# Dao-AILab/flash-attention

Hardware: AMD Instinct MI355X
Metric: attention_fwd_tflops (higher is better)
Workload: dtype bf16; 1 GPU; BASELINE config 3: B=4 H=32 S=4096 D=128 bf16 causal, forward (flash_attn_func path, fa_fwd via C ABI); batch=4, heads=32, seqlen=4096, head_dim=128, causal=True, parallelism=replicas x1

## Files before the change

flash-attention_amd/csrc/fa_fwd_w64.hip:

```cpp
#include <cstddef>
#include <cstdio>
#include <cstdlib>
#include <type_traits>

#include "fa_device.h"
#include "fa_kernel_params.h"
#include "fa_launch.h"
#include "fa_fwd_w64_regs.h"
#define FA_W64_CLOB FA_W64_ACC_CLOBBERS
#include "fa_w64_asm.h"


#define FA_W64_AH 3
#define FA_W64_KDMA_G0 0
#define FA_W64_KDMA_GS 2
#define FA_W64_VDMA_G0 1
#define FA_W64_VDMA_GS 2

namespace fa {

template <int D> FA_DEVINL constexpr int k_swz_w(int row) { return D == 128 ? (row & 15) : ((row >> 1) & 7); }
template <int D> FA_DEVINL constexpr int v_swz_w(int row) { return D == 128 ? (row & 3) : ((row >> 1) & 1); }

#define FA_W64_MFMA(E_) (std::is_same<E_, __bf16>::value ? "v_mfma_f32_32x32x16_bf16" : "v_mfma_f32_32x32x16_f16")
constexpr int W64_Q_BASE = 128;
template <typename E, int F> FA_DEVINL void mfma_s_first(f32x16& d, u32x4 a, const f32x16& c) {
  if constexpr (std::is_same<E, __bf16>::value)
    asm volatile("v_mfma_f32_32x32x16_bf16 %0, %1, a[%c3:%c4], %2" : "=&v"(d) : "v"(a), "v"(c), "i"(W64_Q_BASE + 4 * F), "i"(W64_Q_BASE + 4 * F + 3) : FA_W64_ACC_CLOBBERS);
  else
    asm volatile("v_mfma_f32_32x32x16_f16 %0, %1, a[%c3:%c4], %2" : "=&v"(d) : "v"(a), "v"(c), "i"(W64_Q_BASE + 4 * F), "i"(W64_Q_BASE + 4 * F + 3) : FA_W64_ACC_CLOBBERS);
}
template <typename E, int F> FA_DEVINL void mfma_s_acc(f32x16& d, u32x4 a) {
  if constexpr (std::is_same<E, __bf16>::value)
    asm volatile("v_mfma_f32_32x32x16_bf16 %0, %1, a[%c2:%c3], %0" : "+v"(d) : "v"(a), "i"(W64_Q_BASE + 4 * F), "i"(W64_Q_BASE + 4 * F + 3) : FA_W64_ACC_CLOBBERS);
  else
    asm volatile("v_mfma_f32_32x32x16_f16 %0, %1, a[%c2:%c3], %0" : "+v"(d) : "v"(a), "i"(W64_Q_BASE + 4 * F), "i"(W64_Q_BASE + 4 * F + 3) : FA_W64_ACC_CLOBBERS);
}
template <typename E, int T> FA_DEVINL void mfma_o_acc(u32x4 a, u32x4 b) {
  if constexpr (std::is_same<E, __bf16>::value)
    asm volatile("v_mfma_f32_32x32x16_bf16 a[%c2:%c3], %0, %1, a[%c2:%c3]" : : "v"(a), "v"(b), "i"(16 * T), "i"(16 * T + 15) : FA_W64_ACC_CLOBBERS);
  else
    asm volatile("v_mfma_f32_32x32x16_f16 a[%c2:%c3], %0, %1, a[%c2:%c3]" : : "v"(a), "v"(b), "i"(16 * T), "i"(16 * T + 15) : FA_W64_ACC_CLOBBERS);
}
template <typename E, int D, int FEAT = 0, bool PAGED = false, bool DENSE = false>
__global__ void __launch_bounds__(256, 1) fa_fwd_w64_kernel(const FwdK p) {
  constexpr bool ALIBI = FEAT == FEAT_ALIBI;
  static_assert(!PAGED || FEAT == 0, "the paged variant serves plain attention");
  static_assert(!DENSE || (FEAT == 0 && !PAGED), "the dense variant serves plain attention on contiguous keys / values");
  constexpr bool SOFTCAP = FEAT == FEAT_CAP;
  constexpr bool DROP = FEAT == FEAT_DROP;
  constexpr bool DESC = ALIBI;
  static_assert(FEAT == 0 || FEAT == FEAT_ALIBI || FEAT == FEAT_CAP || FEAT == FEAT_DROP, "feature variants of this schedule: none, causal ALiBi, softcap, dropout");
  using T = ElemTraits<E>;
  using V8 = typename T::v8;
  constexpr int NW = 4, QB = 2, BM = NW * 64, BN = 64, CPR = D / 8;
  constexpr int ROW_BYTES = D * 2;
  constexpr int TILE_BYTES = BN * ROW_BYTES;
  constexpr int KS = D / 16;
  constexpr int DB = D / 32;
  static_assert(D == 64 || D == 128, "head dims built natively: 64, 128");
  constexpr float kLn2 = 0.6931471805599453f;

  extern __shared__ __attribute__((aligned(16))) char smem[];
  char FA_LDS* lds = (char FA_LDS*)smem;
  constexpr int STAGE_BYTES = BM * (ROW_BYTES + 16);
  constexpr int Q_OFF = (4 * TILE_BYTES > STAGE_BYTES ? 4 * TILE_BYTES : STAGE_BYTES + 1023) / 1024 * 1024;

  const int tid = threadIdx.x;
  const int lane = tid & 63;
  const int wave = __builtin_amdgcn_readfirstlane(tid >> 6);
  const int hi = lane >> 5, qi = lane & 31;

  const int d_row = lane / CPR, d_pc = lane % CPR;
  constexpr int RPD = 1024 / ROW_BYTES;

// ... 252 lines not shown
  {
    q_in_lds = -1;
    if (nxt_id_ok && fill_blk(nxt)) {
      asm volatile("s_waitcnt lgkmcnt(0)" ::: "memory");
      qn_srd = q_srd_of(nxt); qn_done = 0;
      qn_per_iter = n_tiles >= QDMA ? 1 : n_tiles >= QDMA / 2 ? 2 : n_tiles >= QDMA / 4 ? 4 : QDMA;
      if (n_tiles == 0) { dma_q(qn_srd); lds_dma_wait_all(); qn_done = QDMA; }
      q_in_lds = vb + (int)gridDim.x;
    }
  }
  auto q_trickle = [&]() __attribute__((always_inline)) {
    if (qn_done < QDMA) {
#pragma unroll 1
      for (int j = 0; j < qn_per_iter; ++j) dma_q_piece(qn_srd, qn_done + j);
      qn_done += qn_per_iter;
    }
  };

  const int kbase = qi * ROW_BYTES + ((hi ^ k_swz_w<D>(qi)) << 4);
  const int tr_i = lane & 15, tr_half = (lane >> 4) & 1;
  const int tr_rr = tr_i >> 2, tr_cc = tr_i & 3;
  const int vbase = (4 * hi + tr_rr) * ROW_BYTES + (v_swz_w<D>(tr_rr) << 6) + tr_half * 32 + tr_cc * 8;
  int ka[KS], va[DB];
#pragma unroll
  for (int ks = 0; ks < KS; ++ks) ka[ks] = kbase ^ (ks << 5);
#pragma unroll
  for (int db = 0; db < DB; ++db) va[db] = vbase ^ (db << 6);

  {
    u32x4 zf = {0u, 0u, 0u, 0u};
    asm volatile("" : "+v"(zf));
    acc_zero_tuples_mfma<0>(zf, std::make_integer_sequence<int, 2 * DB>{});
  }
  float m_run[QB], l_run[QB][2], o_lag[QB];
  float thr_l[QB];
  float capc = 0.f, cap_m2c = 0.f, capoff[QB] = {0.f, 0.f};
  if constexpr (SOFTCAP) {
    capc = __builtin_bit_cast(float, __builtin_amdgcn_readfirstlane(__builtin_bit_cast(int, p.softcap * 1.4426950408889634f)));
    cap_m2c = -2.f * capc;
    capoff[0] = capc; capoff[1] = capc;
  }
  unsigned drop_kr[7] = {0u, 0u, 0u, 0u, 0u, 0u, 0u}, drop_thr = 255u, drop_row[QB] = {0u, 0u};
  if constexpr (DROP) {
    const unsigned k0_ = (unsigned)__builtin_amdgcn_readfirstlane((int)drop_bh_key(p.rng, b * p.h + h));
#pragma unroll
    for (int r = 0; r < 7; ++r) drop_kr[r] = k0_ + (unsigned)r * 0x9E3779B9u;
    drop_thr = (unsigned)__builtin_amdgcn_readfirstlane((int)p.drop_thr8);
#pragma unroll
    for (int qb = 0; qb < QB; ++qb) drop_row[qb] = (unsigned)(w_row0 + 32 * qb + qi);
  }
  constexpr float kCapTiny = 7.888609052210118e-31f;
  unsigned long long lag_mask = 0ull;
  f32x16 negm[QB];
  int arel[QB] = {0, 0};
  if constexpr (ALIBI) {
#pragma unroll
    for (int qb = 0; qb < QB; ++qb) arel[qb] = 4 * hi - (w_row0 + 32 * qb + qi) - shift;
  }
  const float ainc = slope2 * 32.f;
  f32x16 sA[QB], sB[QB];
  u32x4 pfA[QB][2], pfB[QB][2];
#pragma unroll
  for (int qb = 0; qb < QB; ++qb) {
    m_run[qb] = -INFINITY; l_run[qb][0] = 0.f; l_run[qb][1] = 0.f; o_lag[qb] = 1.f; thr_l[qb] = -INFINITY;
#pragma unroll
    for (int r = 0; r < 16; ++r) { negm[qb][r] = ALIBI ? slope2 * (float)(arel[qb] + step_key(0) + acc_row(r, 0)) : 0.f; sA[qb][r] = -INFINITY; sB[qb][r] = -INFINITY; }
#pragma unroll
    for (int t = 0; t < 2; ++t) { pfA[qb][t] = u32x4{0u, 0u, 0u, 0u}; pfB[qb][t] = u32x4{0u, 0u, 0u, 0u}; }
  }

  auto rescale = [&](auto qbc, bool grow, float tmax, f32x16& s_nxt) __attribute__((always_inline)) {
    constexpr int qb = decltype(qbc)::value;
    const float m_base = (m_run[qb] == -INFINITY) ? 0.f : m_run[qb];
    const float m_upd = grow ? (tmax + m_base) : m_run[qb];
    const float m_safe = (m_upd == -INFINITY) ? 0.f : m_upd;
    const float alpha = (grow && m_run[qb] != -INFINITY) ? fast_exp2(m_run[qb] - m_safe) : 1.f;
    const float delta = m_safe - m_base;
    m_run[qb] = m_upd;
    thr_l[qb] = grow ? thr : thr_l[qb];
    l_run[qb][0] *= alpha;
    l_run[qb][1] *= alpha;
    const float neg = -m_safe;
    if constexpr (SOFTCAP) capoff[qb] = capc - m_safe;
#pragma unroll
    for (int r = 0; r < (SOFTCAP ? 0 : 16); ++r) {
      float sv = s_nxt[r], nv = negm[qb][r];
      if constexpr (ALIBI) asm volatile("v_sub_f32 %0, %0, %2\n\tv_sub_f32 %1, %1, %2" : "+v"(sv), "+v"(nv) : "v"(delta), "v"(neg));
      else asm volatile("v_sub_f32 %0, %0, %2\n\tv_mov_b32 %1, %3" : "+v"(sv), "+v"(nv) : "v"(delta), "v"(neg));
      s_nxt[r] = sv;
      negm[qb][r] = nv;
    }
    if (lag_mask != 0ull) acc_scale_range<16 * DB * qb>(o_lag[qb], std::make_integer_sequence<int, 16 * DB>{});
    o_lag[qb] = alpha;
  };
  auto decide_and_rescale = [&](const float (&tmax)[QB], f32x16 (&s_nxt)[QB]) __attribute__((always_inline)) {
    unsigned long long grow_mask;
    asm volatile("v_cmp_gt_f32 vcc, %1, %2\n\tv_cmp_gt_f32 %0, %3, %4\n\ts_or_b64 %0, %0, vcc"
                 : "=&s"(grow_mask) : "v"(tmax[0]), "v"(thr_l[0]), "v"(tmax[1]), "v"(thr_l[1]) : "vcc");
    if (__builtin_expect((grow_mask | lag_mask) != 0ull, 0)) {
      const bool g0 = tmax[0] > thr_l[0], g1 = tmax[1] > thr_l[1];
      mfma_drain_acc();
      rescale(ICw<0>{}, g0, tmax[0], s_nxt[0]);
      rescale(ICw<1>{}, g1, tmax[1], s_nxt[1]);
      lag_mask = __builtin_amdgcn_ballot_w64(o_lag[0] != 1.f || o_lag[1] != 1.f) != 0ull ? ~0ull : 0ull;
    }
  };
  auto set_mask = [&](int i_step) __attribute__((always_inline)) {
    const int k0m = step_key(i_step);
    float ninf = -INFINITY;
    asm volatile("" : "+v"(ninf));
    static_for<QB>([&](auto mqc) __attribute__((always_inline)) {
      constexpr int mq = decltype(mqc)::value;
      float nb = (SOFTCAP || m_run[mq] == -INFINITY) ? 0.f : -m_run[mq];
      const int rel_hi = min(lim_hi[mq] - k0m - 4 * hi, 31), rel_lo = max(lim_lo[mq] - k0m - 4 * hi, 0);
      const unsigned ones = (rel_hi - rel_lo >= 31) ? 0xffffffffu : ((2u << ((rel_hi - rel_lo) & 31)) - 1u);
      unsigned bits = (rel_hi >= rel_lo) ? (ones << (rel_lo & 31)) : 0u;
      if constexpr (ALIBI) nb += slope2 * (float)(arel[mq] + k0m);
      asm volatile("" : "+v"(nb), "+v"(bits));
#pragma unroll
      for (int r = 0; r < 16; r += 4) {
        float n0 = negm[mq][r], n1 = negm[mq][r + 1], n2 = negm[mq][r + 2], n3 = negm[mq][r + 3];
        unsigned t0, t1;
        if constexpr (ALIBI) {
          const float v0 = nb + slope2 * (float)acc_row(r, 0), v1 = nb + slope2 * (float)acc_row(r + 1, 0);
          const float v2 = nb + slope2 * (float)acc_row(r + 2, 0), v3 = nb + slope2 * (float)acc_row(r + 3, 0);
          asm volatile("v_bfe_i32 %4, %6, %c11, 1\n\tv_bfe_i32 %5, %6, %c12, 1\n\tv_bfi_b32 %0, %4, %7, %15\n\tv_bfi_b32 %1, %5, %8, %15\n\t"
                       "v_bfe_i32 %4, %6, %c13, 1\n\tv_bfe_i32 %5, %6, %c14, 1\n\tv_bfi_b32 %2, %4, %9, %15\n\tv_bfi_b32 %3, %5, %10, %15"
                       : "+v"(n0), "+v"(n1), "+v"(n2), "+v"(n3), "=&v"(t0), "=&v"(t1)
                       : "v"(bits), "v"(v0), "v"(v1), "v"(v2), "v"(v3), "i"(acc_row(r, 0)), "i"(acc_row(r + 1, 0)), "i"(acc_row(r + 2, 0)), "i"(acc_row(r + 3, 0)),
                         "v"(ninf));
        } else {
          asm volatile("v_bfe_i32 %4, %6, %c9, 1\n\tv_bfe_i32 %5, %6, %c10, 1\n\tv_bfi_b32 %0, %4, %7, %8\n\tv_bfi_b32 %1, %5, %7, %8\n\t"
                       "v_bfe_i32 %4, %6, %c11, 1\n\tv_bfe_i32 %5, %6, %c12, 1\n\tv_bfi_b32 %2, %4, %7, %8\n\tv_bfi_b32 %3, %5, %7, %8"
                       : "+v"(n0), "+v"(n1), "+v"(n2), "+v"(n3), "=&v"(t0), "=&v"(t1)
                       : "v"(bits), "v"(nb), "v"(ninf), "i"(acc_row(r, 0)), "i"(acc_row(r + 1, 0)), "i"(acc_row(r + 2, 0)), "i"(acc_row(r + 3, 0)));
        }
        negm[mq][r] = n0; negm[mq][r + 1] = n1; negm[mq][r + 2] = n2; negm[mq][r + 3] = n3;
      }
    });
  };
  auto clear_mask = [&](int i_next) __attribute__((always_inline)) {
    static_for<QB>([&](auto mqc) __attribute__((always_inline)) {
      constexpr int mq = decltype(mqc)::value;
      float nb = (SOFTCAP || m_run[mq] == -INFINITY) ? 0.f : -m_run[mq];
      if constexpr (ALIBI) nb += slope2 * (float)(arel[mq] + step_key(i_next));
      asm volatile("" : "+v"(nb));
#pragma unroll
      for (int r = 0; r < 16; ++r) {
        float nv = negm[mq][r];
        float val = nb;
        if constexpr (ALIBI) val = nb + slope2 * (float)acc_row(r, 0);
        asm volatile("v_mov_b32 %0, %1" : "+v"(nv) : "v"(val));
        negm[mq][r] = nv;
      }
    });
  };
  auto fast_step = [&](auto halfc, auto parc, f32x16 (&s_cur)[QB], f32x16 (&s_nxt)[QB],
                       const u32x4 (&pf_prev)[QB][2], u32x4 (&pf_cur)[QB][2], const u32x4& dma_srd, const unsigned (&dma_off)[DPW],
                       unsigned dma_toff, unsigned dma_dst, u32x4 (&kfr)[FA_W64_AH + 1], int drop_k0q = 0, auto modec = ICw<0>{}) __attribute__((always_inline)) {
    constexpr int half = decltype(halfc)::value, par = decltype(parc)::value;
    constexpr int MODE = decltype(modec)::value;
    constexpr bool DO_QK = MODE <= 2, DO_P = MODE == 0 || MODE == 2 || MODE == 3, DO_PV = MODE == 0 || MODE >= 3;
    constexpr int QKG = 2 * KS, PVG = 4 * DB, NG = QKG + PVG;
    auto drop_gap = [](int G, int r) constexpr { return ((7 * G + r) * (NG - 2)) / 56; };
    constexpr bool drop_in_time = [&]() constexpr {
      constexpr int cpg = 16 / PVG > 0 ? 16 / PVG : 1;
      for (int G = 0; G < 8; ++G) if (drop_gap(G, 6) >= QKG + (2 * G) / cpg) return false;
      return true;
    }();
    static_assert(!DROP || drop_in_time, "a Philox word is finished before its first element is packed");
    unsigned ph_c0[8], ph_c1[8];
    constexpr int KOFF = par * TILE_BYTES + half * 32 * ROW_BYTES;
    constexpr int VOFF = (2 + (par ^ 1)) * TILE_BYTES + half * 32 * ROW_BYTES;
    constexpr int AH = FA_W64_AH, RING = AH + 1;
    constexpr int NF = KS + 2 * DB;
    static_assert(RING == FA_W64_AH + 1, "the K fragment ring is the caller's (carried from a first step to its second step)");
    s16x4 vlo[RING], vhi[RING];
    auto rd_frag = [&](int f) __attribute__((always_inline)) {
      if (f < KS) {
        if constexpr (DO_QK) kfr[f % RING] = *(const u32x4 FA_LDS*)(unsigned long)(unsigned)(ka[f] + KOFF);
      } else if (f < NF && DO_PV) {
        const int op = f - KS;
        const char FA_LDS* a0 = (const char FA_LDS*)(unsigned long)(unsigned)(va[op % DB] + VOFF + (16 * (op / DB)) * ROW_BYTES);
        vlo[f % RING] = lds_read_tr16(a0);
        vhi[f % RING] = lds_read_tr16(a0 + 8 * ROW_BYTES);
      }
    };
    auto el_end = [](int x) constexpr { return SOFTCAP ? 32 : x <= QKG ? (24 * x) / QKG : (24 + ((x - QKG) * 16) / PVG > 32 ? 32 : 24 + ((x - QKG) * 16) / PVG); };
    float pe[QB][16];
    auto cap_a = [](int x) constexpr {
      if (x <= 0) return 0;
      if (x <= QKG) return (20 * x) / QKG;
// ... 49 lines not shown
        }
      }
      if constexpr (DROP) {
#pragma unroll
        for (int G = 0; G < 8; ++G)
#pragma unroll
          for (int r = 0; r < 7; ++r)
            if (drop_gap(G, r) == x) {
              if (r == 0) { ph_c0[G] = (unsigned)(drop_k0q + 2 * (G & 3)) + (unsigned)hi; ph_c1[G] = drop_row[G >> 2]; }
              const unsigned mh = __umulhi(0xD256D193u, ph_c0[G]), ml = 0xD256D193u * ph_c0[G];
              unsigned x3;
              asm("v_bitop3_b32 %0, %1, %2, %3 bitop3:0x96" : "=v"(x3) : "v"(mh), "s"(drop_kr[r]), "v"(ph_c1[G]));
              ph_c0[G] = x3;
              ph_c1[G] = ml;
            }
      }
      if constexpr (SOFTCAP) {
#pragma unroll
        for (int e = cap_a(x - 2); e < cap_a(x - 1); ++e) {
          const int eq = e >> 4, r = e & 15;
          pe[eq][r] = fast_exp2(cap_arg[e]);
          l_run[eq][r & 1] += pe[eq][r];
        }
#pragma unroll
        for (int e = cap_a(x - 1); e < cap_a(x); ++e) cap_arg[e] = __builtin_fmaf(__builtin_amdgcn_rcpf(cap_d[e]), cap_m2c, cap_a1[e]);
#pragma unroll
        for (int e = cap_a(x); e < cap_a(x + 1); ++e) {
          const float yv = s_cur[e >> 4][e & 15];
          cap_a1[e] = __builtin_fmaf(yv, kCapTiny, capoff[e >> 4]);
          cap_d[e] = fast_exp2(yv) + 1.f;
        }
      }
#pragma unroll
      for (int e = (DO_P ? el_end(x) : 32); e < (DO_P ? el_end(x + 1) : 32); ++e) {
        const int eq = e >> 4, r = e & 15;
        pe[eq][r] = fast_exp2(s_cur[eq][r]);
        l_run[eq][r & 1] += pe[eq][r];
      }
      if constexpr (x >= QKG) {
        constexpr int y = x - QKG;
        constexpr int CPG = 16 / PVG > 0 ? 16 / PVG : 1;
#pragma unroll
        for (int c = (DO_P ? y * CPG : 16); c < (y + 1) * CPG && c < 16; ++c) {
          const int j = c >> 2, m = c & 3, cq = j >> 1, t = j & 1;
          using V2 = __attribute__((ext_vector_type(2))) E;
          V2 pr;
          float pv0 = pe[cq][8 * t + 2 * m], pv1 = pe[cq][8 * t + 2 * m + 1];
          if constexpr (DROP) {
            const int r0 = 8 * t + 2 * m;
            const unsigned w = ph_c0[4 * cq + (r0 >> 2)];
            pv0 = (((w >> (8 * (r0 & 3))) & 0xffu) > drop_thr) ? 0.f : pv0;
            pv1 = (((w >> (8 * ((r0 + 1) & 3))) & 0xffu) > drop_thr) ? 0.f : pv1;
          }
          pr[0] = (E)pv0;
          pr[1] = (E)pv1;
          unsigned pw = __builtin_bit_cast(unsigned, pr);
          asm volatile("" : "+v"(pw));
          pf_cur[cq][t][m] = pw;
        }
#pragma unroll
        for (int mq = (DO_QK ? 0 : QB); mq < QB; ++mq) {
          const int g0 = tree_g0(mq);
          if (y >= g0 && y < g0 + 8 / UPG) {
#pragma unroll
            for (int u = (y - g0) * UPG; u < (y - g0 + 1) * UPG; ++u)
              if (u == 7 && UPG == 1) {
                float t_in = tmax[mq], t_out, t_cp;
                asm volatile("v_max_f32 %0, %2, %3\n\tv_mov_b32 %1, %0" : "=&v"(t_out), "=v"(t_cp) : "v"(t_in), "v"(s_nxt[mq][15]));
                tmax[mq] = t_out; tcopy[mq] = t_cp;
              } else
              tmax[mq] = u == 0 ? vmax3(s_nxt[mq][0], s_nxt[mq][1], s_nxt[mq][2])
                                : u < 7 ? vmax3(tmax[mq], s_nxt[mq][2 * u + 1], s_nxt[mq][2 * u + 2]) : vmax2(tmax[mq], s_nxt[mq][15]);
          }
          if (y == hm_gap(mq) - 1 && UPG != 1) asm volatile("v_mov_b32 %0, %1" : "=v"(tcopy[mq]) : "v"(tmax[mq]));
          if (y == hm_gap(mq)) {
            if constexpr (!DO_PV) asm volatile("s_nop 1\n\tv_permlane32_swap_b32 %0, %1\n\tv_max_f32 %0, %0, %1" : "+v"(tmax[mq]), "+v"(tcopy[mq]));
            else asm volatile("v_permlane32_swap_b32 %0, %1\n\tv_max_f32 %0, %0, %1" : "+v"(tmax[mq]), "+v"(tcopy[mq]));
          }
          if constexpr (SOFTCAP) {
            constexpr int last = PVG - 1;
            const int g1 = hm_gap(mq) + 1 < last ? hm_gap(mq) + 1 : last, g2 = hm_gap(mq) + 2 < last ? hm_gap(mq) + 2 : last, g3 = hm_gap(mq) + 3 < last ? hm_gap(mq) + 3 : last;
            if (y == g1) cap_g[mq] = fast_exp2(tmax[mq]) + 1.f;
            if (y == g2) cap_g[mq] = __builtin_fmaf(__builtin_amdgcn_rcpf(cap_g[mq]), cap_m2c, capoff[mq]);
            if (y == g3) cap_gt[mq] = __builtin_fmaf(tmax[mq], kCapTiny, cap_g[mq]);
          }
        }
      }
      if constexpr (half == 0 && x >= NG - AH && DO_QK) {
        constexpr int fn = x - (NG - AH);
        kfr[fn % RING] = *(const u32x4 FA_LDS*)(unsigned long)(unsigned)(ka[fn] + par * TILE_BYTES + 32 * ROW_BYTES);
      }
      __builtin_amdgcn_sched_barrier(0);
    });
#pragma unroll
    for (int mq = 0; mq < QB; ++mq)
      if (hm_gap(mq) >= PVG && DO_QK) tmax[mq] = vhalf_max(tmax[mq]);
    static_assert(!SOFTCAP || QB + 8 / UPG < PVG - 1, "softcap: the capped maximum is made inside the gaps");
    if constexpr (SOFTCAP) { tmax[0] = cap_gt[0]; tmax[1] = cap_gt[1]; }
    if constexpr (MODE != 4) decide_and_rescale(tmax, s_nxt);
  };

  int u_first = n_tiles + 1, u_last = n_tiles, p_lo = n_tiles + 1, p_hi = n_tiles;
  if (wave_valid && n_tiles > 0) {
    const int a_lo = max(0, (w_kmin - key_base) >> 5);
    const int a_hi = min(n_steps - 1, (w_kmax - key_base) >> 5);
    if (a_hi >= a_lo) {
      u_first = a_lo >> 1; u_last = min(n_tiles, (a_hi + 2) >> 1);
      const int f_lo = max(0, (w_full_lo - key_base + 31) >> 5);
      const int f_hi = (w_full_hi - 31 - key_base) >> 5;
      p_lo = max(u_first, (f_lo + 1) >> 1);
      p_hi = min(u_last, (f_hi - 1) >> 1);
      if constexpr (DESC) {
        const int t_lo = a_lo >> 1, t_hi = a_hi >> 1, pl_t = (f_lo + 1) >> 1, ph_t = (f_hi - 1) >> 1;
        u_first = n_tiles - 1 - t_hi; u_last = n_tiles - t_lo;
        p_lo = max(u_first, n_tiles - 1 - ph_t);
        p_hi = min(u_last, n_tiles - 1 - pl_t);
      }
      if (p_hi < p_lo) { p_lo = u_last + 1; p_hi = u_last; }
    }
  }
  u_first = __builtin_amdgcn_readfirstlane(u_first); u_last = __builtin_amdgcn_readfirstlane(u_last);
  const unsigned wave_dst = (unsigned)(wave * DPW * 1024);
  auto iter_end = [&]() __attribute__((always_inline)) {
    lds_dma_wait_all();
    __syncthreads();
  };
  const int m_lo = __builtin_amdgcn_readfirstlane(p_lo), m_hi = __builtin_amdgcn_readfirstlane(p_hi);
  const unsigned step_k = (unsigned)(BN * 2) * (unsigned)p.k_rs, step_v = (unsigned)(BN * 2) * (unsigned)p.v_rs;
  const int nmin_s = __builtin_amdgcn_readfirstlane(n_min), nts_s = __builtin_amdgcn_readfirstlane(n_tiles);
  int pg_blk_k = 0, pg_tin_k = 0, pg_blk_v = 0, pg_tin_v = 0, pg_page_n = 0, pg_tin_n = 0;
  auto pg_enter = [&](int u) __attribute__((always_inline)) {
    if constexpr (PAGED) {
      const int nv = n_min + u, nk = nv + 1, nn = nv + 2;
      pg_tin_v = nv % pg_tpp; pg_blk_v = page_entry(nv / pg_tpp);
      pg_tin_k = nk % pg_tpp; pg_blk_k = page_entry(nk / pg_tpp);
      pg_page_n = nn / pg_tpp; pg_tin_n = nn - pg_page_n * pg_tpp;
    }
  };
  auto step_pair = [&](auto parc, int u, auto pmc) __attribute__((always_inline)) {
    constexpr int par = decltype(parc)::value, PM = decltype(pmc)::value;
    using M0 = ICw<(PM == 1 ? 1 : PM == 2 ? 3 : 0)>; using M1 = ICw<(PM == 1 ? 2 : PM == 2 ? 4 : 0)>;
    q_trickle();
    u32x4 kring[FA_W64_AH + 1];
    const int us = __builtin_amdgcn_readfirstlane(u);
    unsigned dst_k = (unsigned)((par ^ 1) * TILE_BYTES) + wave_dst, dst_v = (unsigned)((2 + par) * TILE_BYTES) + wave_dst;
    unsigned tk_ = (unsigned)(nmin_s + (DESC ? nts_s - 2 - us : us + 1)) * step_k, tv_ = (unsigned)(nmin_s + (DESC ? nts_s - 1 - us : us)) * step_v;
    int im32 = ((us - m_lo) | (m_hi - us)) >> 31;
    dst_k = __builtin_amdgcn_readfirstlane(dst_k); dst_v = __builtin_amdgcn_readfirstlane(dst_v);
    im32 = __builtin_amdgcn_readfirstlane(im32);
    u32x4 srd_k = k_srd, srd_v = v_srd;
    if constexpr (PAGED) {
      const int bk = __builtin_amdgcn_readfirstlane(pg_blk_k), tk = __builtin_amdgcn_readfirstlane(pg_tin_k);
      const int bv = __builtin_amdgcn_readfirstlane(pg_blk_v), tv = __builtin_amdgcn_readfirstlane(pg_tin_v);
      const int pn = __builtin_amdgcn_readfirstlane(pg_page_n), tn = __builtin_amdgcn_readfirstlane(pg_tin_n);
      srd_k = tile_srd(ICw<0>{}, bk, tk, nmin_s + us + 1);
      srd_v = tile_srd(ICw<1>{}, bv, tv, nmin_s + us);
      tk_ = 0u; tv_ = 0u;
      pg_blk_v = bk; pg_tin_v = tk;
      pg_blk_k = page_entry(pn); pg_tin_k = tn;
      const bool wrap = tn + 1 == pg_tpp;
      pg_tin_n = wrap ? 0 : tn + 1;
      pg_page_n = wrap ? pn + 1 : pn;
    }
    asm volatile("" : "+s"(tk_), "+s"(tv_), "+s"(dst_k), "+s"(dst_v), "+s"(im32));
    auto masked = [&]() __attribute__((always_inline)) { int c = im32; asm volatile("" : "+s"(c)); return c != 0; };
    if constexpr (PM != 2) { if (__builtin_expect(masked(), 0)) set_mask(2 * u); }
    fast_step(ICw<0>{}, parc, sA, sB, pfA, pfB, srd_k, koff_l, tk_, dst_k, kring, DROP ? step_key(2 * us - 1) >> 2 : 0, M0{});
    if constexpr (PM != 2) { if (__builtin_expect(masked(), 0)) set_mask(2 * u + 1); }
    fast_step(ICw<1>{}, parc, sB, sA, pfB, pfA, srd_v, voff_l, tv_, dst_v, kring, DROP ? step_key(2 * us) >> 2 : 0, M1{});
    if constexpr (PM != 2) {
      if (__builtin_expect(masked(), 0)) {
        int to_last = FEAT == 0 ? u_last - 1 - us : 1;
        asm volatile("" : "+s"(to_last));
        if (to_last != 0) clear_mask(2 * u + 2);
      }
    }
    iter_end();
  };
  auto idle_iter = [&](int u) __attribute__((always_inline)) {
    q_trickle();
    dma_tile(ICw<0>{}, (u & 1) ^ 1, tile_of(u + 1)); dma_tile(ICw<1>{}, u & 1, tile_of(u));
    iter_end();
  };
  if (n_tiles > 0) {
    const bool active = u_first <= u_last;
    const int ua = active ? (u_first & ~1) : n_tiles + 1;
    int u = 0;
#pragma unroll 1
    for (; u < ua; ++u) idle_iter(u);
    if (active) {
      pg_enter(u);
      if constexpr (ALIBI) { if (u > 0) clear_mask(2 * u); }
      if constexpr (FEAT == 0) {
        step_pair(ICw<0>{}, u, ICw<1>{}); ++u;
#pragma unroll 1
        for (;;) {
          if (u >= u_last) break;
          step_pair(ICw<1>{}, u, ICw<0>{}); ++u;
          if (u >= u_last) break;
          step_pair(ICw<0>{}, u, ICw<0>{}); ++u;
        }
        if (u & 1) step_pair(ICw<1>{}, u, ICw<2>{}); else step_pair(ICw<0>{}, u, ICw<2>{});
        ++u;
      } else {
#pragma unroll 1
        for (;;) {
          step_pair(ICw<0>{}, u, ICw<0>{}); ++u;
          if (u > u_last) break;
          step_pair(ICw<1>{}, u, ICw<0>{}); ++u;
          if (u > u_last) break;
        }
      }
    }
#pragma unroll 1
    for (; u <= n_tiles; ++u) idle_iter(u);
  }

  if (wave_valid) {
  mfma_drain_acc();
  u32x4 o_srd;
  {
    const int rows = min(BM, sq - m0);
    const unsigned long long a = (unsigned long long)(op + (int64_t)m0 * p.o_rs);
    const unsigned lo = __builtin_amdgcn_readfirstlane((unsigned)a);
    const unsigned hi16 = __builtin_amdgcn_readfirstlane((unsigned)(a >> 32)) & 0xffffu;
    const unsigned nr = __builtin_amdgcn_readfirstlane((unsigned)(((unsigned long long)(rows - 1) * (unsigned long long)p.o_rs + D) * 2ull));
    o_srd = u32x4{lo, hi16, nr, 0x00020000u};
  }
  static_for<QB>([&](auto qbc) __attribute__((always_inline)) {
    constexpr int qb = decltype(qbc)::value;
    f32x16 o_v[DB];
    static_for<DB>([&](auto dbc) __attribute__((always_inline)) {
      constexpr int db = decltype(dbc)::value;
      acc_read_tuple<16 * (qb * DB + db)>(o_v[db]);
    });
    const float l_tot = half_sum(l_run[qb][0] + l_run[qb][1]);
    const bool dead = (l_tot == 0.f) || (l_tot != l_tot);
    const float inv = (dead ? 1.f : 1.f / l_tot) * o_lag[qb] * (DROP ? p.rp_keep : 1.f);
    const int row0 = w_row0 + 32 * qb;
    if (row0 < sq) {
      {
        using V4 = typename T::v4;
        constexpr int RS = ROW_BYTES + 16, RPI = 64 / CPR;
        char FA_LDS* stage = lds + (wave * 64 + qb * 32) * RS;
#pragma unroll
        for (int db = 0; db < DB; ++db)
#pragma unroll
          for (int g = 0; g < 4; ++g) {
            V4 ov;
#pragma unroll
            for (int jj = 0; jj < 4; ++jj) ov[jj] = (E)(o_v[db][4 * g + jj] * inv);
            *reinterpret_cast<V4 FA_LDS*>(stage + qi * RS + (32 * db + 8 * g + 4 * hi) * 2) = ov;
          }
        unsigned lane_off = (unsigned)(((wave * 64 + lane / CPR) * (int)p.o_rs + (lane % CPR) * 8) * 2);
        asm volatile("" : "+v"(lane_off));
#pragma unroll
        for (int i = 0; i < 32 / RPI; ++i) {
          const u32x4 x = *reinterpret_cast<const u32x4 FA_LDS*>(stage + (i * RPI + lane / CPR) * RS + (lane % CPR) * 16);
          const unsigned soff = __builtin_amdgcn_readfirstlane((unsigned)((qb * 32 + i * RPI) * (int)p.o_rs * 2));
          asm volatile("buffer_store_dwordx4 %0, %1, %2, %3 offen" : : "v"(x), "v"(lane_off), "s"(o_srd), "s"(soff) : "memory");
        }
        asm volatile("s_waitcnt lgkmcnt(0)" ::: "memory");
      }
      const int my_row = row0 + qi;
      if (my_row < sq && hi == 0) lsep[my_row] = dead ? INFINITY : (m_run[qb] * kLn2 + __logf(l_tot));
    }
  });
  }
  }
}

template <typename E, int D, int FEAT = 0, bool PAGED = false, bool DENSE = false>
static int launch_fwd_w64_t(const FwdK& p, hipStream_t stream) {
  if constexpr (FEAT == 0 && !PAGED && !DENSE) {
    if (!p.cu_q && !p.cu_k && !p.seqused_q && !p.seqused_k && !p.leftpad_k && !p.kv_batch_idx && !p.work_list && p.wl < 0)
      return launch_fwd_w64_t<E, D, 0, false, true>(p, stream);
  }
  constexpr int STAGE = 256 * (D * 2 + 16);
  constexpr int smem = ((4 * 64 * D * 2 > STAGE ? 4 * 64 * D * 2 : STAGE + 1023) / 1024 * 1024) + 256 * D * 2;
  auto kern = fa_fwd_w64_kernel<E, D, FEAT, PAGED, DENSE>;
  static std::atomic<unsigned long long> attr_mask{0};
  if (ensure_dyn_lds(attr_mask, (const void*)kern, smem, true) != 0) return -1;
  const long long total = p.work_list ? (long long)p.work_bound * p.h : units_grid(p.n_units, p.unit_size);
  if (total <= 0) return 0;
  FwdK pp = p;
  fwd_w64_reciprocals(pp);
  long long grid = total;
  const int cus = device_cu_count();
  const bool balanced = p.wr < 0 || (p.unit_size > 1 && (cus / 8) % p.unit_size == 0);
  if (!p.work_list && cus >= 8 && total > cus && balanced && knobs().w64_persist != 0) {
    grid = cus / 8 * 8;
    pp.persist_total = (int)total;
  }
  FA_LAUNCH(kern, dim3((unsigned)grid), dim3(256), smem, stream, pp);
  if (hipGetLastError() != hipSuccess) return -1;
  LastSchedule& ls = last_schedule();
  ls.fwd_kernel = 3; ls.fwd_nw = 4; ls.fwd_feat = FEAT; ls.fwd_splits = 1; ls.fwd_list = p.work_list != nullptr; ls.d = D;
  ls.bf16 = std::is_same<E, __bf16>::value;
// ... 81 lines not shown
```

flash-attention_amd/csrc/fa_fwd_w64_regs.h:

```cpp
#pragma once
#define FA_W64_ACC_CLOBBERS "a0", "a1", "a2", "a3", "a4", "a5", "a6", "a7", "a8", "a9", "a10", "a11", "a12", "a13", \
  "a14", "a15", "a16", "a17", "a18", "a19", "a20", "a21", "a22", "a23", "a24", "a25", "a26", "a27", "a28", "a29", \
  "a30", "a31", "a32", "a33", "a34", "a35", "a36", "a37", "a38", "a39", "a40", "a41", "a42", "a43", "a44", "a45", \
  "a46", "a47", "a48", "a49", "a50", "a51", "a52", "a53", "a54", "a55", "a56", "a57", "a58", "a59", "a60", "a61", \
  "a62", "a63", "a64", "a65", "a66", "a67", "a68", "a69", "a70", "a71", "a72", "a73", "a74", "a75", "a76", "a77", \
  "a78", "a79", "a80", "a81", "a82", "a83", "a84", "a85", "a86", "a87", "a88", "a89", "a90", "a91", "a92", "a93", \
  "a94", "a95", "a96", "a97", "a98", "a99", "a100", "a101", "a102", "a103", "a104", "a105", "a106", "a107", "a108", \
  "a109", "a110", "a111", "a112", "a113", "a114", "a115", "a116", "a117", "a118", "a119", "a120", "a121", "a122", \
  "a123", "a124", "a125", "a126", "a127", "a128", "a129", "a130", "a131", "a132", "a133", "a134", "a135", "a136", \
  "a137", "a138", "a139", "a140", "a141", "a142", "a143", "a144", "a145", "a146", "a147", "a148", "a149", "a150", \
  "a151", "a152", "a153", "a154", "a155", "a156", "a157", "a158", "a159", "a160", "a161", "a162", "a163", "a164", \
  "a165", "a166", "a167", "a168", "a169", "a170", "a171", "a172", "a173", "a174", "a175", "a176", "a177", "a178", \
  "a179", "a180", "a181", "a182", "a183", "a184", "a185", "a186", "a187", "a188", "a189", "a190", "a191"
#define FA_W64_ACC_CLOBBERS_256 FA_W64_ACC_CLOBBERS, \
  "a192", "a193", "a194", "a195", "a196", "a197", "a198", "a199", "a200", "a201", "a202", "a203", "a204", \
  "a205", "a206", "a207", "a208", "a209", "a210", "a211", "a212", "a213", "a214", "a215", "a216", "a217", \
  "a218", "a219", "a220", "a221", "a222", "a223", "a224", "a225", "a226", "a227", "a228", "a229", "a230", \
  "a231", "a232", "a233", "a234", "a235", "a236", "a237", "a238", "a239", "a240", "a241", "a242", "a243", \
  "a244", "a245", "a246", "a247", "a248", "a249", "a250", "a251", "a252", "a253", "a254", "a255"
```

Measured before the change: 1096 TFLOP/s.

## Keep softmax state in AGPRs and fold causal mask handling into rescale branch

```diff
diff --git a/flash-attention_amd/csrc/fa_fwd_w64.hip b/flash-attention_amd/csrc/fa_fwd_w64.hip
--- a/flash-attention_amd/csrc/fa_fwd_w64.hip
+++ b/flash-attention_amd/csrc/fa_fwd_w64.hip
@@ -7,7 +7,7 @@
 #include "fa_kernel_params.h"
 #include "fa_launch.h"
 #include "fa_fwd_w64_regs.h"
-#define FA_W64_CLOB FA_W64_ACC_CLOBBERS
+#define FA_W64_CLOB FA_W64_FWD_CLOBBERS
 #include "fa_w64_asm.h"
 
 
@@ -24,23 +24,24 @@
 
 #define FA_W64_MFMA(E_) (std::is_same<E_, __bf16>::value ? "v_mfma_f32_32x32x16_bf16" : "v_mfma_f32_32x32x16_f16")
 constexpr int W64_Q_BASE = 128;
+constexpr int W64_M_BASE = 192, W64_LAG_BASE = 194;
 template <typename E, int F> FA_DEVINL void mfma_s_first(f32x16& d, u32x4 a, const f32x16& c) {
   if constexpr (std::is_same<E, __bf16>::value)
-    asm volatile("v_mfma_f32_32x32x16_bf16 %0, %1, a[%c3:%c4], %2" : "=&v"(d) : "v"(a), "v"(c), "i"(W64_Q_BASE + 4 * F), "i"(W64_Q_BASE + 4 * F + 3) : FA_W64_ACC_CLOBBERS);
+    asm volatile("v_mfma_f32_32x32x16_bf16 %0, %1, a[%c3:%c4], %2" : "=&v"(d) : "v"(a), "v"(c), "i"(W64_Q_BASE + 4 * F), "i"(W64_Q_BASE + 4 * F + 3) : FA_W64_CLOB);
   else
-    asm volatile("v_mfma_f32_32x32x16_f16 %0, %1, a[%c3:%c4], %2" : "=&v"(d) : "v"(a), "v"(c), "i"(W64_Q_BASE + 4 * F), "i"(W64_Q_BASE + 4 * F + 3) : FA_W64_ACC_CLOBBERS);
+    asm volatile("v_mfma_f32_32x32x16_f16 %0, %1, a[%c3:%c4], %2" : "=&v"(d) : "v"(a), "v"(c), "i"(W64_Q_BASE + 4 * F), "i"(W64_Q_BASE + 4 * F + 3) : FA_W64_CLOB);
 }
 template <typename E, int F> FA_DEVINL void mfma_s_acc(f32x16& d, u32x4 a) {
   if constexpr (std::is_same<E, __bf16>::value)
-    asm volatile("v_mfma_f32_32x32x16_bf16 %0, %1, a[%c2:%c3], %0" : "+v"(d) : "v"(a), "i"(W64_Q_BASE + 4 * F), "i"(W64_Q_BASE + 4 * F + 3) : FA_W64_ACC_CLOBBERS);
+    asm volatile("v_mfma_f32_32x32x16_bf16 %0, %1, a[%c2:%c3], %0" : "+v"(d) : "v"(a), "i"(W64_Q_BASE + 4 * F), "i"(W64_Q_BASE + 4 * F + 3) : FA_W64_CLOB);
   else
-    asm volatile("v_mfma_f32_32x32x16_f16 %0, %1, a[%c2:%c3], %0" : "+v"(d) : "v"(a), "i"(W64_Q_BASE + 4 * F), "i"(W64_Q_BASE + 4 * F + 3) : FA_W64_ACC_CLOBBERS);
+    asm volatile("v_mfma_f32_32x32x16_f16 %0, %1, a[%c2:%c3], %0" : "+v"(d) : "v"(a), "i"(W64_Q_BASE + 4 * F), "i"(W64_Q_BASE + 4 * F + 3) : FA_W64_CLOB);
 }
 template <typename E, int T> FA_DEVINL void mfma_o_acc(u32x4 a, u32x4 b) {
   if constexpr (std::is_same<E, __bf16>::value)
-    asm volatile("v_mfma_f32_32x32x16_bf16 a[%c2:%c3], %0, %1, a[%c2:%c3]" : : "v"(a), "v"(b), "i"(16 * T), "i"(16 * T + 15) : FA_W64_ACC_CLOBBERS);
+    asm volatile("v_mfma_f32_32x32x16_bf16 a[%c2:%c3], %0, %1, a[%c2:%c3]" : : "v"(a), "v"(b), "i"(16 * T), "i"(16 * T + 15) : FA_W64_CLOB);
   else
-    asm volatile("v_mfma_f32_32x32x16_f16 a[%c2:%c3], %0, %1, a[%c2:%c3]" : : "v"(a), "v"(b), "i"(16 * T), "i"(16 * T + 15) : FA_W64_ACC_CLOBBERS);
+    asm volatile("v_mfma_f32_32x32x16_f16 a[%c2:%c3], %0, %1, a[%c2:%c3]" : : "v"(a), "v"(b), "i"(16 * T), "i"(16 * T + 15) : FA_W64_CLOB);
 }
 template <typename E, int D, int FEAT = 0, bool PAGED = false, bool DENSE = false>
 __global__ void __launch_bounds__(256, 1) fa_fwd_w64_kernel(const FwdK p) {
@@ -359,7 +360,12 @@
     asm volatile("" : "+v"(zf));
     acc_zero_tuples_mfma<0>(zf, std::make_integer_sequence<int, 2 * DB>{});
   }
-  float m_run[QB], l_run[QB][2], o_lag[QB];
+  constexpr bool ACC_STATE = !ALIBI;
+  float l_run[QB][2], m_run_v[QB] = {-INFINITY, -INFINITY}, o_lag_v[QB] = {1.f, 1.f};
+  auto m_get = [&](auto qbc) __attribute__((always_inline)) { constexpr int qb = decltype(qbc)::value; if constexpr (ACC_STATE) return acc_read<W64_M_BASE + qb>(); else return m_run_v[qb]; };
+  auto m_set = [&](auto qbc, float x) __attribute__((always_inline)) { constexpr int qb = decltype(qbc)::value; if constexpr (ACC_STATE) acc_write<W64_M_BASE + qb>(x); else m_run_v[qb] = x; };
+  auto lag_get = [&](auto qbc) __attribute__((always_inline)) { constexpr int qb = decltype(qbc)::value; if constexpr (ACC_STATE) return acc_read<W64_LAG_BASE + qb>(); else return o_lag_v[qb]; };
+  auto lag_set = [&](auto qbc, float x) __attribute__((always_inline)) { constexpr int qb = decltype(qbc)::value; if constexpr (ACC_STATE) acc_write<W64_LAG_BASE + qb>(x); else o_lag_v[qb] = x; };
   float thr_l[QB];
   float capc = 0.f, cap_m2c = 0.f, capoff[QB] = {0.f, 0.f};
   if constexpr (SOFTCAP) {
@@ -377,7 +383,7 @@
     for (int qb = 0; qb < QB; ++qb) drop_row[qb] = (unsigned)(w_row0 + 32 * qb + qi);
   }
   constexpr float kCapTiny = 7.888609052210118e-31f;
-  unsigned long long lag_mask = 0ull;
+  unsigned long long pending = 0ull;
   f32x16 negm[QB];
   int arel[QB] = {0, 0};
   if constexpr (ALIBI) {
@@ -389,21 +395,24 @@
   u32x4 pfA[QB][2], pfB[QB][2];
 #pragma unroll
   for (int qb = 0; qb < QB; ++qb) {
-    m_run[qb] = -INFINITY; l_run[qb][0] = 0.f; l_run[qb][1] = 0.f; o_lag[qb] = 1.f; thr_l[qb] = -INFINITY;
+    l_run[qb][0] = 0.f; l_run[qb][1] = 0.f; thr_l[qb] = -INFINITY;
 #pragma unroll
     for (int r = 0; r < 16; ++r) { negm[qb][r] = ALIBI ? slope2 * (float)(arel[qb] + step_key(0) + acc_row(r, 0)) : 0.f; sA[qb][r] = -INFINITY; sB[qb][r] = -INFINITY; }
 #pragma unroll
     for (int t = 0; t < 2; ++t) { pfA[qb][t] = u32x4{0u, 0u, 0u, 0u}; pfB[qb][t] = u32x4{0u, 0u, 0u, 0u}; }
   }
 
-  auto rescale = [&](auto qbc, bool grow, float tmax, f32x16& s_nxt) __attribute__((always_inline)) {
+  m_set(ICw<0>{}, -INFINITY); m_set(ICw<1>{}, -INFINITY); lag_set(ICw<0>{}, 1.f); lag_set(ICw<1>{}, 1.f);
+
+  auto rescale = [&](auto qbc, bool grow, bool lagged, float tmax, f32x16& s_nxt) __attribute__((always_inline)) {
     constexpr int qb = decltype(qbc)::value;
-    const float m_base = (m_run[qb] == -INFINITY) ? 0.f : m_run[qb];
-    const float m_upd = grow ? (tmax + m_base) : m_run[qb];
+    const float m_old = m_get(qbc);
+    const float m_base = (m_old == -INFINITY) ? 0.f : m_old;
+    const float m_upd = grow ? (tmax + m_base) : m_old;
     const float m_safe = (m_upd == -INFINITY) ? 0.f : m_upd;
-    const float alpha = (grow && m_run[qb] != -INFINITY) ? fast_exp2(m_run[qb] - m_safe) : 1.f;
+    const float alpha = (grow && m_old != -INFINITY) ? fast_exp2(m_old - m_safe) : 1.f;
     const float delta = m_safe - m_base;
-    m_run[qb] = m_upd;
+    m_set(qbc, m_upd);
     thr_l[qb] = grow ? thr : thr_l[qb];
     l_run[qb][0] *= alpha;
     l_run[qb][1] *= alpha;
@@ -417,19 +426,35 @@
       s_nxt[r] = sv;
       negm[qb][r] = nv;
     }
-    if (lag_mask != 0ull) acc_scale_range<16 * DB * qb>(o_lag[qb], std::make_integer_sequence<int, 16 * DB>{});
-    o_lag[qb] = alpha;
-  };
-  auto decide_and_rescale = [&](const float (&tmax)[QB], f32x16 (&s_nxt)[QB]) __attribute__((always_inline)) {
+    if (lagged) acc_scale_range<16 * DB * qb>(lag_get(qbc), std::make_integer_sequence<int, 16 * DB>{});
+    lag_set(qbc, alpha);
+    return alpha;
+  };
+  auto decide_and_rescale = [&](const float (&tmax)[QB], f32x16 (&s_nxt)[QB], auto&& mask_work) __attribute__((always_inline)) {
     unsigned long long grow_mask;
     asm volatile("v_cmp_gt_f32 vcc, %1, %2\n\tv_cmp_gt_f32 %0, %3, %4\n\ts_or_b64 %0, %0, vcc"
                  : "=&s"(grow_mask) : "v"(tmax[0]), "v"(thr_l[0]), "v"(tmax[1]), "v"(thr_l[1]) : "vcc");
-    if (__builtin_expect((grow_mask | lag_mask) != 0ull, 0)) {
-      const bool g0 = tmax[0] > thr_l[0], g1 = tmax[1] > thr_l[1];
-      mfma_drain_acc();
-      rescale(ICw<0>{}, g0, tmax[0], s_nxt[0]);
-      rescale(ICw<1>{}, g1, tmax[1], s_nxt[1]);
-      lag_mask = __builtin_amdgcn_ballot_w64(o_lag[0] != 1.f || o_lag[1] != 1.f) != 0ull ? ~0ull : 0ull;
+    if constexpr (ALIBI) {
+      if (__builtin_expect((grow_mask | pending) != 0ull, 0)) {
+        const bool g0 = tmax[0] > thr_l[0], g1 = tmax[1] > thr_l[1];
+        mfma_drain_acc();
+        rescale(ICw<0>{}, g0, pending != 0ull, tmax[0], s_nxt[0]);
+        rescale(ICw<1>{}, g1, pending != 0ull, tmax[1], s_nxt[1]);
+        pending = __builtin_amdgcn_ballot_w64(o_lag_v[0] != 1.f || o_lag_v[1] != 1.f) != 0ull ? ~0ull : 0ull;
+      }
+    } else
+    if (__builtin_expect((grow_mask | pending) != 0ull, 0)) {
+      unsigned lag = (unsigned)(pending >> 32), mk = (unsigned)pending;
+      asm volatile("" : "+s"(lag), "+s"(mk));
+      if (grow_mask != 0ull || lag != 0u) {
+        const bool g0 = tmax[0] > thr_l[0], g1 = tmax[1] > thr_l[1];
+        mfma_drain_acc();
+        const float a0 = rescale(ICw<0>{}, g0, lag != 0u, tmax[0], s_nxt[0]);
+        const float a1 = rescale(ICw<1>{}, g1, lag != 0u, tmax[1], s_nxt[1]);
+        lag = __builtin_amdgcn_ballot_w64(a0 != 1.f || a1 != 1.f) != 0ull ? ~0u : 0u;
+      }
+      if (__builtin_expect(mk != 0u, 0)) mask_work();
+      pending = ((unsigned long long)lag << 32) | (unsigned long long)mk;
     }
   };
   auto set_mask = [&](int i_step) __attribute__((always_inline)) {
@@ -438,7 +463,8 @@
     asm volatile("" : "+v"(ninf));
     static_for<QB>([&](auto mqc) __attribute__((always_inline)) {
       constexpr int mq = decltype(mqc)::value;
-      float nb = (SOFTCAP || m_run[mq] == -INFINITY) ? 0.f : -m_run[mq];
+      const float m_cur = SOFTCAP ? 0.f : m_get(mqc);
+      float nb = (SOFTCAP || m_cur == -INFINITY) ? 0.f : -m_cur;
       const int rel_hi = min(lim_hi[mq] - k0m - 4 * hi, 31), rel_lo = max(lim_lo[mq] - k0m - 4 * hi, 0);
       const unsigned ones = (rel_hi - rel_lo >= 31) ? 0xffffffffu : ((2u << ((rel_hi - rel_lo) & 31)) - 1u);
       unsigned bits = (rel_hi >= rel_lo) ? (ones << (rel_lo & 31)) : 0u;
@@ -469,7 +495,8 @@
   auto clear_mask = [&](int i_next) __attribute__((always_inline)) {
     static_for<QB>([&](auto mqc) __attribute__((always_inline)) {
       constexpr int mq = decltype(mqc)::value;
-      float nb = (SOFTCAP || m_run[mq] == -INFINITY) ? 0.f : -m_run[mq];
+      const float m_cur = SOFTCAP ? 0.f : m_get(mqc);
+      float nb = (SOFTCAP || m_cur == -INFINITY) ? 0.f : -m_cur;
       if constexpr (ALIBI) nb += slope2 * (float)(arel[mq] + step_key(i_next));
       asm volatile("" : "+v"(nb));
 #pragma unroll
@@ -484,7 +511,7 @@
   };
   auto fast_step = [&](auto halfc, auto parc, f32x16 (&s_cur)[QB], f32x16 (&s_nxt)[QB],
                        const u32x4 (&pf_prev)[QB][2], u32x4 (&pf_cur)[QB][2], const u32x4& dma_srd, const unsigned (&dma_off)[DPW],
-                       unsigned dma_toff, unsigned dma_dst, u32x4 (&kfr)[FA_W64_AH + 1], int drop_k0q = 0, auto modec = ICw<0>{}) __attribute__((always_inline)) {
+                       unsigned dma_toff, unsigned dma_dst, u32x4 (&kfr)[FA_W64_AH + 1], int drop_k0q, auto modec, auto&& mask_work) __attribute__((always_inline)) {
     constexpr int half = decltype(halfc)::value, par = decltype(parc)::value;
     constexpr int MODE = decltype(modec)::value;
     constexpr bool DO_QK = MODE <= 2, DO_P = MODE == 0 || MODE == 2 || MODE == 3, DO_PV = MODE == 0 || MODE >= 3;
@@ -600,10 +627,11 @@
         }
       }
 #pragma unroll
-      for (int e = (DO_P ? el_end(x) : 32); e < (DO_P ? el_end(x + 1) : 32); ++e) {
-        const int eq = e >> 4, r = e & 15;
-        pe[eq][r] = fast_exp2(s_cur[eq][r]);
-        l_run[eq][r & 1] += pe[eq][r];
+      for (int e = (DO_P ? el_end(x) : 32); e < (DO_P ? el_end(x + 1) : 32); ++e) pe[e >> 4][e & 15] = fast_exp2(s_cur[e >> 4][e & 15]);
+      if constexpr (DO_P && !SOFTCAP) {
+        auto la = [&](int g) constexpr { return g <= 0 ? 0 : el_end(g - 1) == 32 ? 32 : el_end(g) > 2 ? el_end(g) - 2 : 0; };
+#pragma unroll
+        for (int e = la(x); e < la(x + 1); ++e) l_run[e >> 4][e & 1] += pe[e >> 4][e & 15];
       }
       if constexpr (x >= QKG) {
         constexpr int y = x - QKG;
@@ -665,7 +693,7 @@
       if (hm_gap(mq) >= PVG && DO_QK) tmax[mq] = vhalf_max(tmax[mq]);
     static_assert(!SOFTCAP || QB + 8 / UPG < PVG - 1, "softcap: the capped maximum is made inside the gaps");
     if constexpr (SOFTCAP) { tmax[0] = cap_gt[0]; tmax[1] = cap_gt[1]; }
-    if constexpr (MODE != 4) decide_and_rescale(tmax, s_nxt);
+    if constexpr (MODE != 4) decide_and_rescale(tmax, s_nxt, mask_work);
   };
 
   int u_first = n_tiles + 1, u_last = n_tiles, p_lo = n_tiles + 1, p_hi = n_tiles;
@@ -694,6 +722,8 @@
     __syncthreads();
   };
   const int m_lo = __builtin_amdgcn_readfirstlane(p_lo), m_hi = __builtin_amdgcn_readfirstlane(p_hi);
+  const int mk_hi = (FEAT == 0 && m_hi + 1 >= u_last) ? m_hi : m_hi - 1;
+  auto masked_it = [&](int ui) __attribute__((always_inline)) { return (((ui - m_lo) | (m_hi - ui)) >> 31) != 0; };
   const unsigned step_k = (unsigned)(BN * 2) * (unsigned)p.k_rs, step_v = (unsigned)(BN * 2) * (unsigned)p.v_rs;
   const int nmin_s = __builtin_amdgcn_readfirstlane(n_min), nts_s = __builtin_amdgcn_readfirstlane(n_tiles);
   int pg_blk_k = 0, pg_tin_k = 0, pg_blk_v = 0, pg_tin_v = 0, pg_page_n = 0, pg_tin_n = 0;
@@ -713,7 +743,8 @@
     const int us = __builtin_amdgcn_readfirstlane(u);
     unsigned dst_k = (unsigned)((par ^ 1) * TILE_BYTES) + wave_dst, dst_v = (unsigned)((2 + par) * TILE_BYTES) + wave_dst;
     unsigned tk_ = (unsigned)(nmin_s + (DESC ? nts_s - 2 - us : us + 1)) * step_k, tv_ = (unsigned)(nmin_s + (DESC ? nts_s - 1 - us : us)) * step_v;
-    int im32 = ((us - m_lo) | (m_hi - us)) >> 31;
+    constexpr bool COLD_MASKS = !ALIBI;
+    int im32 = PM == 2 ? 0 : ((us - m_lo) | ((COLD_MASKS ? mk_hi : m_hi) - us)) >> 31;
     dst_k = __builtin_amdgcn_readfirstlane(dst_k); dst_v = __builtin_amdgcn_readfirstlane(dst_v);
     im32 = __builtin_amdgcn_readfirstlane(im32);
     u32x4 srd_k = k_srd, srd_v = v_srd;
@@ -731,18 +762,23 @@
       pg_page_n = wrap ? pn + 1 : pn;
     }
     asm volatile("" : "+s"(tk_), "+s"(tv_), "+s"(dst_k), "+s"(dst_v), "+s"(im32));
+    if constexpr (COLD_MASKS) pending = (pending & 0xffffffff00000000ull) | (unsigned long long)(unsigned)im32;
     auto masked = [&]() __attribute__((always_inline)) { int c = im32; asm volatile("" : "+s"(c)); return c != 0; };
-    if constexpr (PM != 2) { if (__builtin_expect(masked(), 0)) set_mask(2 * u); }
-    fast_step(ICw<0>{}, parc, sA, sB, pfA, pfB, srd_k, koff_l, tk_, dst_k, kring, DROP ? step_key(2 * us - 1) >> 2 : 0, M0{});
-    if constexpr (PM != 2) { if (__builtin_expect(masked(), 0)) set_mask(2 * u + 1); }
-    fast_step(ICw<1>{}, parc, sB, sA, pfB, pfA, srd_v, voff_l, tv_, dst_v, kring, DROP ? step_key(2 * us) >> 2 : 0, M1{});
-    if constexpr (PM != 2) {
-      if (__builtin_expect(masked(), 0)) {
-        int to_last = FEAT == 0 ? u_last - 1 - us : 1;
-        asm volatile("" : "+s"(to_last));
-        if (to_last != 0) clear_mask(2 * u + 2);
-      }
-    }
+    if constexpr (!COLD_MASKS && PM != 2) { if (__builtin_expect(masked(), 0)) set_mask(2 * u); }
+    fast_step(ICw<0>{}, parc, sA, sB, pfA, pfB, srd_k, koff_l, tk_, dst_k, kring, DROP ? step_key(2 * us - 1) >> 2 : 0, M0{}, [&]() __attribute__((always_inline)) {
+      if constexpr (COLD_MASKS && PM != 2) { if (masked_it(us)) set_mask(2 * us + 1); }
+    });
+    if constexpr (!COLD_MASKS && PM != 2) { if (__builtin_expect(masked(), 0)) set_mask(2 * u + 1); }
+    fast_step(ICw<1>{}, parc, sB, sA, pfB, pfA, srd_v, voff_l, tv_, dst_v, kring, DROP ? step_key(2 * us) >> 2 : 0, M1{}, [&]() __attribute__((always_inline)) {
+      if constexpr (COLD_MASKS && PM != 2) {
+        const int un = us + 1;
+        if (FEAT == 0 ? un != u_last : un <= u_last) {
+          if (masked_it(un)) set_mask(2 * un);
+          else if (masked_it(us)) clear_mask(2 * un);
+        }
+      }
+    });
+    if constexpr (!COLD_MASKS && PM != 2) { if (__builtin_expect(masked(), 0)) clear_mask(2 * u + 2); }
     iter_end();
   };
   auto idle_iter = [&](int u) __attribute__((always_inline)) {
@@ -759,15 +795,17 @@
     if (active) {
       pg_enter(u);
       if constexpr (ALIBI) { if (u > 0) clear_mask(2 * u); }
+      if constexpr (!ALIBI) { if (masked_it(u)) set_mask(2 * u); }
       if constexpr (FEAT == 0) {
         step_pair(ICw<0>{}, u, ICw<1>{}); ++u;
+        int uu = __builtin_amdgcn_readfirstlane(u);
 #pragma unroll 1
-        for (;;) {
-          if (u >= u_last) break;
-          step_pair(ICw<1>{}, u, ICw<0>{}); ++u;
-          if (u >= u_last) break;
-          step_pair(ICw<0>{}, u, ICw<0>{}); ++u;
+        for (int pairs = (u_last - uu) >> 1; pairs > 0; --pairs) {
+          step_pair(ICw<1>{}, uu, ICw<0>{}); ++uu;
+          step_pair(ICw<0>{}, uu, ICw<0>{}); ++uu;
         }
+        if (uu < u_last) { step_pair(ICw<1>{}, uu, ICw<0>{}); ++uu; }
+        u = uu;
         if (u & 1) step_pair(ICw<1>{}, u, ICw<2>{}); else step_pair(ICw<0>{}, u, ICw<2>{});
         ++u;
       } else {
@@ -804,7 +842,7 @@
     });
     const float l_tot = half_sum(l_run[qb][0] + l_run[qb][1]);
     const bool dead = (l_tot == 0.f) || (l_tot != l_tot);
-    const float inv = (dead ? 1.f : 1.f / l_tot) * o_lag[qb] * (DROP ? p.rp_keep : 1.f);
+    const float inv = (dead ? 1.f : 1.f / l_tot) * lag_get(qbc) * (DROP ? p.rp_keep : 1.f);
     const int row0 = w_row0 + 32 * qb;
     if (row0 < sq) {
       {
@@ -826,12 +864,12 @@
         for (int i = 0; i < 32 / RPI; ++i) {
           const u32x4 x = *reinterpret_cast<const u32x4 FA_LDS*>(stage + (i * RPI + lane / CPR) * RS + (lane % CPR) * 16);
           const unsigned soff = __builtin_amdgcn_readfirstlane((unsigned)((qb * 32 + i * RPI) * (int)p.o_rs * 2));
-          asm volatile("buffer_store_dwordx4 %0, %1, %2, %3 offen" : : "v"(x), "v"(lane_off), "s"(o_srd), "s"(soff) : "memory");
+          asm volatile("s_nop 4\n\tbuffer_store_dwordx4 %0, %1, %2, %3 offen" : : "v"(x), "v"(lane_off), "s"(o_srd), "s"(soff) : "memory");
         }
         asm volatile("s_waitcnt lgkmcnt(0)" ::: "memory");
       }
       const int my_row = row0 + qi;
-      if (my_row < sq && hi == 0) lsep[my_row] = dead ? INFINITY : (m_run[qb] * kLn2 + __logf(l_tot));
+      if (my_row < sq && hi == 0) lsep[my_row] = dead ? INFINITY : (m_get(qbc) * kLn2 + __logf(l_tot));
     }
   });
   }
diff --git a/flash-attention_amd/csrc/fa_fwd_w64_regs.h b/flash-attention_amd/csrc/fa_fwd_w64_regs.h
--- a/flash-attention_amd/csrc/fa_fwd_w64_regs.h
+++ b/flash-attention_amd/csrc/fa_fwd_w64_regs.h
@@ -12,6 +12,7 @@
   "a151", "a152", "a153", "a154", "a155", "a156", "a157", "a158", "a159", "a160", "a161", "a162", "a163", "a164", \
   "a165", "a166", "a167", "a168", "a169", "a170", "a171", "a172", "a173", "a174", "a175", "a176", "a177", "a178", \
   "a179", "a180", "a181", "a182", "a183", "a184", "a185", "a186", "a187", "a188", "a189", "a190", "a191"
+#define FA_W64_FWD_CLOBBERS FA_W64_ACC_CLOBBERS, "a192", "a193", "a194", "a195"
 #define FA_W64_ACC_CLOBBERS_256 FA_W64_ACC_CLOBBERS, \
   "a192", "a193", "a194", "a195", "a196", "a197", "a198", "a199", "a200", "a201", "a202", "a203", "a204", \
   "a205", "a206", "a207", "a208", "a209", "a210", "a211", "a212", "a213", "a214", "a215", "a216", "a217", \
```

Result: no change. 1098 TFLOP/s, median of 3 (+0.1%).
